# Symb0x76/ChineseChessZero

Measured on AMD Instinct MI355X. Metric: self-play MCTS simulations/sec, higher is better.
Workload: dtype u8 rules / f32 Q (reference CPU path) / f64 PUCT (net: fp16)

## Files before the change

### chinesechesszero_amd/csrc/cczero_conv_g16.h

```cpp
#pragma once
#include "cczero_conv.h"

namespace ccz {

constexpr int kG5Rows = 288;
constexpr int kG5SlabRows = 576;
constexpr int kG5SlabBytes = kG5SlabRows * 64;
constexpr int kG5WBytes = 256 * 64;
constexpr int kG5Ring = 5, kG5Ahead = 3;
constexpr int kG5AOff = kG5Ring * kG5WBytes;
constexpr int kG5Dump = kG5AOff + 2 * kG5SlabBytes;
constexpr int kG5Lds = kG5Dump + 8 * 1024;
constexpr int kG5ERow = 528;
static_assert(kG5Rows * kG5ERow <= kG5Dump, "epilogue image must fit the operand buffers");

struct G5Ctx {
    unsigned char *lds;
    const _Float16 *X, *W;
    unsigned xoff[5];
    unsigned woff;
    int zo[2], zd[2];
    int wave_dst;
    int lane16;
    int wave_dst4;
    int a_off;
    int vb[2];
    int cin, cmask;
};

__host__ __device__ constexpr bool g5_slab_tap(int t) { return t >= 1 && t <= 5; }
constexpr int kG5Split = 7;
__host__ __device__ constexpr int g5_vmcnt(int t) { return 4 + (g5_slab_tap(t) ? 1 : 0) + (g5_slab_tap(t - 1) ? 1 : 0); }

template <int T, int N> __host__ __device__ constexpr bool g5_on_board()
{
    return !((T % 3 == 0 && N == 0) || (T % 3 == 2 && N == 8));
}

__device__ __forceinline__ void g5_zero_ranks(const G5Ctx &c, int buf)
{
    int l16 = c.lane16, zero = 0;
    asm volatile("" : "+v"(l16), "+v"(zero));
    typedef int g5_int4 __attribute__((ext_vector_type(4)));
    const g5_int4 z = {zero, zero, zero, zero};
#pragma unroll
    for (int j = 0; j < 2; ++j) *(g5_int4 *)(c.lds + (l16 + (c.zo[j] + buf * c.zd[j]))) = z;
    asm volatile("s_waitcnt lgkmcnt(0)" ::: "memory");
}

template <int J>
__device__ __forceinline__ void g5_step(const G5Ctx &c, cv_f32x4 (&acc)[4][9], int chunk, int &ring_rd, int &ring_wr,
                                         cv_half8 (&a0)[4], cv_half8 (&a1)[4], cv_half8 (&b)[9])
{
    constexpr int T = J % 9, BUF = J / 9;
    constexpr int Tn = (T + 1) % 9, BUFn = (T == 8) ? 1 - BUF : BUF;
    cv_half8 (&acur)[4] = (J & 1) ? a1 : a0;
    cv_half8 (&anxt)[4] = (J & 1) ? a0 : a1;
    unsigned char *const lds = c.lds;

#define G5_CELL(N)                                                                                                        \
    {                                                                                                                     \
        if constexpr (T % 3 == 2)                                                                                         \
            b[N] = *(const cv_half8 *)(lds + c.vb[BUFn] + (9 + N + 9 * (Tn / 3 - 1)) * 1024);                             \
        if constexpr (g5_on_board<T, N>()) {                                                                              \
            constexpr int NB = N + T % 3 - 1;                                                                             \
            _Pragma("unroll") for (int i = 0; i < 4; ++i)                                                                 \
                acc[i][N] = __builtin_amdgcn_mfma_f32_16x16x32_f16(acur[i], b[NB], acc[i][N], 0, 0, 0);                   \
        }                                                                                                                 \
        __builtin_amdgcn_sched_barrier(0);                                                                                \
    }
#define G5_CELLS(LO, HI)                                                                                                  \
    if constexpr (LO <= 0 && 0 < HI) G5_CELL(0) if constexpr (LO <= 1 && 1 < HI) G5_CELL(1) if constexpr (LO <= 2 && 2 < HI) G5_CELL(2) \
    if constexpr (LO <= 3 && 3 < HI) G5_CELL(3) if constexpr (LO <= 4 && 4 < HI) G5_CELL(4) if constexpr (LO <= 5 && 5 < HI) G5_CELL(5) \
    if constexpr (LO <= 6 && 6 < HI) G5_CELL(6) if constexpr (LO <= 7 && 7 < HI) G5_CELL(7) if constexpr (LO <= 8 && 8 < HI) G5_CELL(8)
    constexpr int T2 = (T + kG5Ahead) % 9;
    const int chunk2 = (chunk + (T + kG5Ahead >= 9 ? 1 : 0)) & c.cmask;
    G5_CELLS(0, 1)
    if constexpr (g5_slab_tap(T)) {
        constexpr int pass = T - 1;
        const int nxt = (chunk + 1) & c.cmask;
        cv_glds16(c.X + (c.xoff[pass] + (unsigned)(nxt * 32)), lds + kG5AOff + (1 - BUF) * kG5SlabBytes + (pass < 4 ? pass * 8192 + c.wave_dst : c.wave_dst4));
        __builtin_amdgcn_sched_barrier(0);
    }
    G5_CELLS(1, 2)
    {
        unsigned wo = c.woff;
        asm volatile("" : "+v"(wo));
        const unsigned o = wo + (unsigned)((T2 + 9 * chunk2) * 8192);
        const unsigned o2 = o + 4096u;
        unsigned char *const d = lds + ring_wr * kG5WBytes + c.wave_dst;
        cv_glds16(c.W + o, d);
        __builtin_amdgcn_sched_barrier(0);
        G5_CELLS(2, 3)
        cv_glds16(c.W + o2, d + 8192);
        __builtin_amdgcn_sched_barrier(0);
    }
    G5_CELLS(3, kG5Split)

    ring_rd = ring_rd + 1 == kG5Ring ? 0 : ring_rd + 1;
    cv_wait_vm<g5_vmcnt(T)>();
    if constexpr (T == 7) g5_zero_ranks(c, 1 - BUF);
    __builtin_amdgcn_sched_barrier(0);
    __builtin_amdgcn_s_barrier();
    __builtin_amdgcn_sched_barrier(0);

    {
        const unsigned char *wa = lds + (ring_rd * kG5WBytes + c.a_off);
#pragma unroll
        for (int i = 0; i < 4; ++i) anxt[i] = *(const cv_half8 *)(wa + i * 1024);
        __builtin_amdgcn_sched_barrier(0);
    }
    G5_CELLS(kG5Split, 9)
    ring_wr = ring_wr + 1 == kG5Ring ? 0 : ring_wr + 1;
#undef G5_CELLS
#undef G5_CELL
}

struct G5Heads {
    const _Float16 *w32;
    const float *b32;
    _Float16 *pol, *val;
    int nb;
};

__device__ __forceinline__ void g5_heads_phase(const unsigned char *lds, int w, int lane, const G5Heads &ha, const long (&board0)[2],
                                               const int (&pos0)[2], bool skip1)
{
    const int r = lane & 15, q4 = lane >> 4;
    cv_half8 a[2][8];
#pragma unroll
    for (int m = 0; m < 2; ++m)
#pragma unroll
        for (int s = 0; s < 8; ++s) a[m][s] = *(const cv_half8 *)(ha.w32 + (m * 16 + r) * 256 + s * 32 + q4 * 8);
    const float4 b0 = *(const float4 *)(ha.b32 + 4 * q4), b1 = *(const float4 *)(ha.b32 + 16 + 4 * q4);
    for (int cell = w; cell < 18; cell += 8) {
        const unsigned char *row = lds + (cell * 16 + r) * kG5ERow + q4 * 16;
        cv_f32x4 acc0, acc1;
        acc0[0] = b0.x; acc0[1] = b0.y; acc0[2] = b0.z; acc0[3] = b0.w;
        acc1[0] = b1.x; acc1[1] = b1.y; acc1[2] = b1.z; acc1[3] = b1.w;
#pragma unroll
        for (int s = 0; s < 8; ++s) {
            const cv_half8 b = *(const cv_half8 *)(row + s * 64);
            acc0 = __builtin_amdgcn_mfma_f32_16x16x32_f16(a[0][s], b, acc0, 0, 0, 0);
            acc1 = __builtin_amdgcn_mfma_f32_16x16x32_f16(a[1][s], b, acc1, 0, 0, 0);
        }
        const int wnr = cell >= 9 ? 1 : 0, n = cell - 9 * wnr;
        const long board = board0[wnr] + r;
        if (board < ha.nb && !(skip1 && wnr)) {
            const int pos = pos0[wnr] + n;
            _Float16 *po = ha.pol + board * 1536 + pos * 17;
            _Float16 *vo = ha.val + board * 640 + pos * 7;
#pragma unroll
            for (int e = 0; e < 4; ++e) po[4 * q4 + e] = (_Float16)fmaxf(acc0[e], 0.0f);
            if (q4 == 0) {
                po[16] = (_Float16)fmaxf(acc1[0], 0.0f);
                vo[0] = (_Float16)fmaxf(acc1[1], 0.0f);
                vo[1] = (_Float16)fmaxf(acc1[2], 0.0f);
                vo[2] = (_Float16)fmaxf(acc1[3], 0.0f);
            } else if (q4 == 1) {
#pragma unroll
                for (int e = 0; e < 4; ++e) vo[3 + e] = (_Float16)fmaxf(acc1[e], 0.0f);
            }
        }
    }
}

__device__ __forceinline__ int g5_live_groups(const int *live_rows, int row0, int cap, int &first)
{
    const int part = row0 & 0xffff, n_parts = row0 >> 16;
    const int G = (*live_rows + 15) >> 4;
    const int per = (G + n_parts - 1) / n_parts;
    first = part * per;
    int live = G - first;
    live = live < 0 ? 0 : (live > per ? per : live);
    return live > cap ? cap : live;
}

template <bool RES, bool HEADS, bool ONE = false>
__device__ __forceinline__ void g5_tile(unsigned char *lds, int blk, int grid, const _Float16 *__restrict__ X, const _Float16 *__restrict__ W,
                                        const float *__restrict__ bias, const _Float16 *R,
                                        _Float16 *Y, int M, int relu, int cin, const int *live_rows, int row0, const G5Heads &ha)
{
    [[maybe_unused]] long first_board = 0;
    const int tid = threadIdx.x, lane = tid & 63;
    const int w = __builtin_amdgcn_readfirstlane(tid >> 6);
    const int r = lane & 15, q4 = lane >> 4;
    const int wm = w & 3, wn = w >> 2;
    int tiles = grid;
    if (live_rows) {
        int first;
        const int live = g5_live_groups(live_rows, row0, M / 1440, first);
        M = live * 1440;
        tiles = live * ((relu & 4) ? 4 : 5);
        if (blk >= tiles) return;
        const long off = (long)first * 1440 * kCvC;
        X += (long)first * 1440 * cin;
        if (!HEADS) Y += off;
        if (RES) R += off;
        first_board = (long)first * 16;
    }
    int tile;
    {
        const int b = blk, x = b & 7, per = tiles >> 3, rem = tiles & 7;
        tile = x * per + (x < rem ? x : rem) + (b >> 3);
    }
    tile = __builtin_amdgcn_readfirstlane((relu & 2) ? tiles - 1 - tile : tile);
    const int mid = relu & 4;
    const int k = mid ? 2 : tile % 5;
    const long p0 = mid ? (long)(tile >> 2) * 1440 + 144 + (long)(tile & 3) * kG5Rows
                        : (long)tile * kG5Rows;
    relu &= 1;

    G5Ctx c;
    c.lds = lds;
    c.X = X;
    c.W = W;
    {
        const int piece[2] = {k == 0 ? 0 : k == 4 ? (w >= 3 ? 3 : 4) : -1, (k == 0 && w == 0) ? 1 : (k == 4 && w == 3) ? 4 : -1};
#pragma unroll
        for (int j = 0; j < 2; ++j) {
            c.zo[j] = __builtin_amdgcn_readfirstlane(piece[j] >= 0 ? kG5AOff + piece[j] * 8192 + w * 1024 : kG5Dump + w * 1024);
            c.zd[j] = __builtin_amdgcn_readfirstlane(piece[j] >= 0 ? kG5SlabBytes : 0);
        }
    }
    c.wave_dst = w * 1024;
    c.lane16 = lane * 16;
    c.wave_dst4 = (w < 4 ? 4 : 3) * 8192 + w * 1024;
    c.cin = cin;
    c.cmask = ONE ? 0 : (cin >> 5) - 1;
    {
#pragma unroll
        for (int it = 0; it < 5; ++it) {
            const int piece = (it < 4 || w < 4) ? it * 512 + tid : 3 * 512 + tid;
            const int sr = piece >> 2, pos = piece & 3;
            const int schunk = pos ^ ((0 - (sr >> 2)) & 3);
            long p = p0 - 144 + sr;
            p = p < 0 ? 0 : (p > (long)M - 1 ? (long)M - 1 : p);
            c.xoff[it] = (unsigned)(p * cin + schunk * 8);
        }
        c.woff = (unsigned)(tid * 8);
    }
#pragma unroll
    for (int it = 0; it < 5; ++it) cv_glds16(X + c.xoff[it], lds + kG5AOff + (it < 4 ? it * 8192 + c.wave_dst : c.wave_dst4));
#pragma unroll
    for (int u = 0; u < kG5Ahead; ++u) {
        const unsigned o = c.woff + (unsigned)(u * 8192);
        unsigned char *d = lds + u * kG5WBytes + c.wave_dst;
        cv_glds16(W + o, d);
        cv_glds16(W + (o + 4096u), d + 8192);
    }
    const int lane1 = r * 64 + ((q4 ^ ((0 - (r >> 2)) & 3)) << 4);
    c.a_off = wm * 4096 + lane1;
    c.vb[0] = kG5AOff + wn * 9 * 1024 + lane1;
    c.vb[1] = c.vb[0] + kG5SlabBytes;

    cv_f32x4 acc[4][9];
#pragma unroll
    for (int i = 0; i < 4; ++i) {
        const float4 bv = *(const float4 *)(bias + wm * 64 + i * 16 + 4 * q4);
#pragma unroll
        for (int n = 0; n < 9; ++n) {
            acc[i][n][0] = bv.x; acc[i][n][1] = bv.y; acc[i][n][2] = bv.z; acc[i][n][3] = bv.w;
        }
    }

    cv_wait_vm<4>();
    g5_zero_ranks(c, 0);
    asm volatile("s_waitcnt lgkmcnt(0)" ::: "memory");
    __builtin_amdgcn_sched_barrier(0);
    __builtin_amdgcn_s_barrier();
    __builtin_amdgcn_sched_barrier(0);

    int ring_rd = 0, ring_wr = kG5Ahead;
    cv_half8 a0[4], a1[4], b[9];
#pragma unroll
    for (int i = 0; i < 4; ++i) a0[i] = *(const cv_half8 *)(lds + c.a_off + i * 1024);
#pragma unroll
    for (int n = 0; n < 9; ++n) b[n] = *(const cv_half8 *)(lds + c.vb[0] + (9 + n - 9) * 1024);
#define G5_S(j) g5_step<j>(c, acc, chunk + (j) / 9, ring_rd, ring_wr, a0, a1, b)
    if constexpr (ONE) {
        const int chunk = 0;
        G5_S(0); G5_S(1); G5_S(2); G5_S(3); G5_S(4); G5_S(5); G5_S(6); G5_S(7); G5_S(8);
    } else {
        for (int chunk = 0; chunk <= c.cmask; chunk += 2) {
            G5_S(0); G5_S(1); G5_S(2); G5_S(3); G5_S(4); G5_S(5); G5_S(6); G5_S(7); G5_S(8);
            G5_S(9); G5_S(10); G5_S(11); G5_S(12); G5_S(13); G5_S(14); G5_S(15); G5_S(16); G5_S(17);
        }
    }
#undef G5_S
    cv_wait_vm<0>();

    __builtin_amdgcn_sched_barrier(0);
    __builtin_amdgcn_s_barrier();
    __builtin_amdgcn_sched_barrier(0);
#pragma unroll
    for (int i = 0; i < 4; ++i) {
        const int col = wm * 64 + i * 16 + 4 * q4;
#pragma unroll
        for (int n = 0; n < 9; ++n) {
            cv_half4 o;
            o[0] = (_Float16)acc[i][n][0];
            o[1] = (_Float16)acc[i][n][1];
            o[2] = (_Float16)acc[i][n][2];
            o[3] = (_Float16)acc[i][n][3];
            *(cv_half4 *)(lds + ((wn * 9 + n) * 16 + r) * kG5ERow + col * 2) = o;
        }
    }
    const int prow = lane >> 5, piece = lane & 31;
    const long pbase = p0 + w * 36 + prow;
    cv_half8 rv[18];
    if (RES) {
#pragma unroll
        for (int it = 0; it < 18; ++it) rv[it] = *(const cv_half8 *)(R + (pbase + it * 2) * kCvC + piece * 8);
    }
    asm volatile("s_waitcnt lgkmcnt(0)" ::: "memory");
    __builtin_amdgcn_sched_barrier(0);
    __builtin_amdgcn_s_barrier();
    __builtin_amdgcn_sched_barrier(0);
    {
        const cv_half8 zero = (cv_half8)(_Float16)0;
        unsigned char *eb = lds + (w * 36 + prow) * kG5ERow + piece * 16;
#pragma unroll
        for (int it = 0; it < 18; ++it) {
            cv_half8 v = *(const cv_half8 *)(eb + it * 2 * kG5ERow);
            if (RES) v = v + rv[it];
            if (relu) v = __builtin_elementwise_max(v, zero);
            if constexpr (HEADS) *(cv_half8 *)(eb + it * 2 * kG5ERow) = v;
            else *(cv_half8 *)(Y + (pbase + it * 2) * kCvC + piece * 8) = v;
        }
    }
    if constexpr (HEADS) {
        asm volatile("s_waitcnt lgkmcnt(0)" ::: "memory");
        __builtin_amdgcn_sched_barrier(0);
        __builtin_amdgcn_s_barrier();
        __builtin_amdgcn_sched_barrier(0);
        const long grp = p0 / 1440;
        const int rank0 = (int)((p0 - grp * 1440) / 144);
        const long board0[2] = {first_board + grp * 16, first_board + grp * 16};
        const int pos0[2] = {rank0 * 9, rank0 * 9 + 9};
        g5_heads_phase(lds, w, lane, ha, board0, pos0, false);
    }
}

template <bool RES>
__global__ __launch_bounds__(512) void k_conv3x3_g16(const _Float16 *__restrict__ X, const _Float16 *__restrict__ W,
                                                         const float *__restrict__ bias, const _Float16 *R,
                                                         _Float16 *Y, int M, int relu, int cin, const int *live_rows, int row0)
{
    __shared__ __attribute__((aligned(16))) unsigned char lds[kG5Lds];
    g5_tile<RES, false>(lds, blockIdx.x, gridDim.x, X, W, bias, R, Y, M, relu, cin, live_rows, row0, G5Heads{});
}

__global__ __launch_bounds__(512) void k_conv3x3_g16_stem(const _Float16 *__restrict__ X, const _Float16 *__restrict__ W,
                                                            const float *__restrict__ bias, _Float16 *Y, int M, int relu, int cin,
                                                            const int *live_rows, int row0)
{
    __shared__ __attribute__((aligned(16))) unsigned char lds[kG5Lds];
    g5_tile<false, false, true>(lds, blockIdx.x, gridDim.x, X, W, bias, nullptr, Y, M, relu, cin, live_rows, row0, G5Heads{});
}

__global__ __launch_bounds__(512) void k_conv3x3_g16_heads(const _Float16 *__restrict__ X, const _Float16 *__restrict__ W,
                                                             const float *__restrict__ bias, const _Float16 *R, _Float16 *Y, int M,
                                                             int relu, int cin, const int *live_rows, int row0, G5Heads ha)
{
    __shared__ __attribute__((aligned(16))) unsigned char lds[kG5Lds];
    if (live_rows) ha.nb = *live_rows;
    g5_tile<true, true>(lds, blockIdx.x, gridDim.x, X, W, bias, R, Y, M, relu, cin, live_rows, row0, ha);
}

__global__ __launch_bounds__(256) void k_pack_conv_weights_g16(const cv_half8 *__restrict__ w, cv_half8 *__restrict__ wp, int cin)
{
    const int n = 256 * 9 * (cin >> 3);
    const int i = blockIdx.x * 256 + threadIdx.x;
    if (i >= n) return;
    const int pos = i & 3, co = (i >> 2) & 255, h = i >> 10, tap = h % 9, c32 = h / 9;
    const int chunk = pos ^ ((0 - (co >> 2)) & 3);
    wp[i] = w[(co * 9 + tap) * (cin >> 3) + c32 * 4 + chunk];
}

}
```

### chinesechesszero_amd/csrc/cczero_conv_g16e.h

```cpp
#pragma once
#include "cczero_conv_g16.h"

namespace ccz {

__host__ __device__ constexpr int g5e_nslab(int h) { return h == 0 ? 2 : h == 1 ? 2 : h == 2 ? 1 : 0; }
__host__ __device__ constexpr int g5e_vmcnt(int h) { return 4 + g5e_nslab(h) + g5e_nslab((h + 5) % 6); }

template <int J>
__device__ __forceinline__ void g5e_step(const G5Ctx &c, cv_f32x4 (&acc)[4][9], int chunk, int &ring_rd, int &ring_wr,
                                          cv_half8 (&a0)[4], cv_half8 (&a1)[4], cv_half8 (&b)[9], int toff)
{
    constexpr int H = J % 6, BUF = J / 6;
    constexpr int Hn = (H + 1) % 6, BUFn = (H == 5) ? 1 - BUF : BUF;
    cv_half8 (&acur)[4] = (J & 1) ? a1 : a0;
    cv_half8 (&anxt)[4] = (J & 1) ? a0 : a1;
    unsigned char *const lds = c.lds;
#define G5E_CELL(N)                                                                                                       \
    {                                                                                                                     \
        if constexpr (H % 3 == 2)                                                                                         \
            b[N] = *(const cv_half8 *)(lds + c.vb[BUFn] + ((Hn / 3) * 9 + N) * 1024);                                     \
        if constexpr (g5_on_board<H, N>()) {                                                                              \
            constexpr int NB = N + H % 3 - 1;                                                                             \
            _Pragma("unroll") for (int i = 0; i < 4; ++i)                                                                 \
                acc[i][N] = __builtin_amdgcn_mfma_f32_16x16x32_f16(acur[i], b[NB], acc[i][N], 0, 0, 0);                   \
        }                                                                                                                 \
        __builtin_amdgcn_sched_barrier(0);                                                                                \
    }
#define G5E_CELLS(LO, HI)                                                                                                 \
    if constexpr (LO <= 0 && 0 < HI) G5E_CELL(0) if constexpr (LO <= 1 && 1 < HI) G5E_CELL(1) if constexpr (LO <= 2 && 2 < HI) G5E_CELL(2) \
    if constexpr (LO <= 3 && 3 < HI) G5E_CELL(3) if constexpr (LO <= 4 && 4 < HI) G5E_CELL(4) if constexpr (LO <= 5 && 5 < HI) G5E_CELL(5) \
    if constexpr (LO <= 6 && 6 < HI) G5E_CELL(6) if constexpr (LO <= 7 && 7 < HI) G5E_CELL(7) if constexpr (LO <= 8 && 8 < HI) G5E_CELL(8)
    constexpr int H2 = (H + kG5Ahead) % 6;
    const int chunk2 = (chunk + (H + kG5Ahead >= 6 ? 1 : 0)) & c.cmask;
    G5E_CELLS(0, 1)
    if constexpr (g5e_nslab(H) > 0) {
        const int nxt = (chunk + 1) & c.cmask;
        constexpr int p0 = H * 2;
        cv_glds16(c.X + (c.xoff[p0] + (unsigned)(nxt * 32)), lds + kG5AOff + (1 - BUF) * kG5SlabBytes + (p0 < 4 ? p0 * 8192 + c.wave_dst : c.wave_dst4));
        if constexpr (g5e_nslab(H) > 1)
            cv_glds16(c.X + (c.xoff[p0 + 1] + (unsigned)(nxt * 32)), lds + kG5AOff + (1 - BUF) * kG5SlabBytes + ((p0 + 1) * 8192 + c.wave_dst));
        __builtin_amdgcn_sched_barrier(0);
    }
    G5E_CELLS(1, 2)
    {
        unsigned wo = c.woff;
        asm volatile("" : "+v"(wo));
        const unsigned o = wo + (unsigned)((H2 + toff + 9 * chunk2) * 8192);
        const unsigned o2 = o + 4096u;
        unsigned char *const d = lds + ring_wr * kG5WBytes + c.wave_dst;
        cv_glds16(c.W + o, d);
        __builtin_amdgcn_sched_barrier(0);
        G5E_CELLS(2, 3)
        cv_glds16(c.W + o2, d + 8192);
        __builtin_amdgcn_sched_barrier(0);
    }
    G5E_CELLS(3, kG5Split)

    ring_rd = ring_rd + 1 == kG5Ring ? 0 : ring_rd + 1;
    cv_wait_vm<g5e_vmcnt(H)>();
    __builtin_amdgcn_sched_barrier(0);
    __builtin_amdgcn_s_barrier();
    __builtin_amdgcn_sched_barrier(0);

    {
        const unsigned char *wa = lds + (ring_rd * kG5WBytes + c.a_off);
#pragma unroll
        for (int i = 0; i < 4; ++i) anxt[i] = *(const cv_half8 *)(wa + i * 1024);
        __builtin_amdgcn_sched_barrier(0);
    }
    G5E_CELLS(kG5Split, 9)
    ring_wr = ring_wr + 1 == kG5Ring ? 0 : ring_wr + 1;
#undef G5E_CELLS
#undef G5E_CELL
}

template <bool RES, bool HEADS>
__device__ __forceinline__ void g5e_tile(unsigned char *lds, int blk, const _Float16 *__restrict__ X, const _Float16 *__restrict__ W,
                                         const float *__restrict__ bias, const _Float16 *R, _Float16 *Y, int M,
                                         int relu, int cin, const int *live_rows, int row0, const G5Heads &ha)
{
    [[maybe_unused]] long first_board = 0;
    const int tid = threadIdx.x, lane = tid & 63;
    const int w = __builtin_amdgcn_readfirstlane(tid >> 6);
    const int r = lane & 15, q4 = lane >> 4;
    const int wm = w & 3, wn = w >> 2;
    int groups = M / 1440;
    if (live_rows) {
        int first;
        groups = g5_live_groups(live_rows, row0, groups, first);
        const long off = (long)first * 1440 * kCvC;
        X += (long)first * 1440 * cin;
        if (!HEADS) Y += off;
        if (RES) R += off;
        first_board = (long)first * 16;
    }
    const int e = __builtin_amdgcn_readfirstlane(blk);
    if (e >= 2 * ((groups + 1) >> 1)) return;
    const int side = e & 1, gA = (e >> 1) * 2;
    const bool dup = gA + 1 >= groups;
    const int gB = dup ? gA : gA + 1;
    const int toff = __builtin_amdgcn_readfirstlane(side ? 0 : 3);
    const long srcA = (long)gA * 1440 + (side ? 8 : 0) * 144;
    const long srcB = (long)gB * 1440 + (side ? 8 : 0) * 144;
    const long outA = (long)gA * 1440 + (side ? 9 : 0) * 144;
    const long outB = (long)gB * 1440 + (side ? 9 : 0) * 144;
    relu &= 1;

    G5Ctx c;
    c.lds = lds;
    c.X = X;
    c.W = W;
    c.wave_dst = w * 1024;
    c.lane16 = lane * 16;
    c.wave_dst4 = (w < 4 ? 4 : 3) * 8192 + w * 1024;
    c.cin = cin;
    c.cmask = (cin >> 5) - 1;
    {
#pragma unroll
        for (int it = 0; it < 5; ++it) {
            const int piece = (it < 4 || w < 4) ? it * 512 + tid : 3 * 512 + tid;
            const int sr = piece >> 2, pos = piece & 3;
            const int schunk = pos ^ ((0 - (sr >> 2)) & 3);
            const long p = sr < 288 ? srcA + sr : srcB + (sr - 288);
            c.xoff[it] = (unsigned)(p * cin + schunk * 8);
        }
        c.woff = (unsigned)(tid * 8);
    }
#pragma unroll
    for (int it = 0; it < 5; ++it) cv_glds16(X + c.xoff[it], lds + kG5AOff + (it < 4 ? it * 8192 + c.wave_dst : c.wave_dst4));
#pragma unroll
    for (int u = 0; u < kG5Ahead; ++u) {
        const unsigned o = c.woff + (unsigned)((u + toff) * 8192);
        unsigned char *d = lds + u * kG5WBytes + c.wave_dst;
        cv_glds16(W + o, d);
        cv_glds16(W + (o + 4096u), d + 8192);
    }
    const int lane1 = r * 64 + ((q4 ^ ((0 - (r >> 2)) & 3)) << 4);
    c.a_off = wm * 4096 + lane1;
    c.vb[0] = kG5AOff + wn * 18 * 1024 + lane1;
    c.vb[1] = c.vb[0] + kG5SlabBytes;

    cv_f32x4 acc[4][9];
#pragma unroll
    for (int i = 0; i < 4; ++i) {
        const float4 bv = *(const float4 *)(bias + wm * 64 + i * 16 + 4 * q4);
#pragma unroll
        for (int n = 0; n < 9; ++n) {
            acc[i][n][0] = bv.x; acc[i][n][1] = bv.y; acc[i][n][2] = bv.z; acc[i][n][3] = bv.w;
        }
    }

    cv_wait_vm<4>();
    __builtin_amdgcn_sched_barrier(0);
    __builtin_amdgcn_s_barrier();
    __builtin_amdgcn_sched_barrier(0);

    int ring_rd = 0, ring_wr = kG5Ahead;
    cv_half8 a0[4], a1[4], b[9];
#pragma unroll
    for (int i = 0; i < 4; ++i) a0[i] = *(const cv_half8 *)(lds + c.a_off + i * 1024);
#pragma unroll
    for (int n = 0; n < 9; ++n) b[n] = *(const cv_half8 *)(lds + c.vb[0] + n * 1024);
    for (int chunk = 0; chunk <= c.cmask; chunk += 2) {
#define G5E_S(j) g5e_step<j>(c, acc, chunk + (j) / 6, ring_rd, ring_wr, a0, a1, b, toff)
        G5E_S(0); G5E_S(1); G5E_S(2); G5E_S(3); G5E_S(4); G5E_S(5);
        G5E_S(6); G5E_S(7); G5E_S(8); G5E_S(9); G5E_S(10); G5E_S(11);
#undef G5E_S
    }
    cv_wait_vm<0>();

    __builtin_amdgcn_sched_barrier(0);
    __builtin_amdgcn_s_barrier();
    __builtin_amdgcn_sched_barrier(0);
#pragma unroll
    for (int i = 0; i < 4; ++i) {
        const int col = wm * 64 + i * 16 + 4 * q4;
#pragma unroll
        for (int n = 0; n < 9; ++n) {
            cv_half4 o;
            o[0] = (_Float16)acc[i][n][0];
            o[1] = (_Float16)acc[i][n][1];
            o[2] = (_Float16)acc[i][n][2];
            o[3] = (_Float16)acc[i][n][3];
            *(cv_half4 *)(lds + ((wn * 9 + n) * 16 + r) * kG5ERow + col * 2) = o;
        }
    }
    const int prow = lane >> 5, piece = lane & 31;
    const long pbase = (w < 4 ? outA : outB) + (w & 3) * 36 + prow;
    const bool store = !(dup && w >= 4);
    cv_half8 rv[18];
    if (RES) {
#pragma unroll
        for (int it = 0; it < 18; ++it) rv[it] = *(const cv_half8 *)(R + (pbase + it * 2) * kCvC + piece * 8);
    }
    asm volatile("s_waitcnt lgkmcnt(0)" ::: "memory");
    __builtin_amdgcn_sched_barrier(0);
    __builtin_amdgcn_s_barrier();
    __builtin_amdgcn_sched_barrier(0);
    if (store) {
        const cv_half8 zero = (cv_half8)(_Float16)0;
        unsigned char *eb = lds + (w * 36 + prow) * kG5ERow + piece * 16;
#pragma unroll
        for (int it = 0; it < 18; ++it) {
            cv_half8 v = *(const cv_half8 *)(eb + it * 2 * kG5ERow);
            if (RES) v = v + rv[it];
            if (relu) v = __builtin_elementwise_max(v, zero);
            if constexpr (HEADS) *(cv_half8 *)(eb + it * 2 * kG5ERow) = v;
            else *(cv_half8 *)(Y + (pbase + it * 2) * kCvC + piece * 8) = v;
        }
    }
    if constexpr (HEADS) {
        asm volatile("s_waitcnt lgkmcnt(0)" ::: "memory");
        __builtin_amdgcn_sched_barrier(0);
        __builtin_amdgcn_s_barrier();
        __builtin_amdgcn_sched_barrier(0);
        const long board0[2] = {first_board + (long)gA * 16, first_board + (long)gB * 16};
        const int pos0[2] = {side ? 81 : 0, side ? 81 : 0};
        g5_heads_phase(lds, w, lane, ha, board0, pos0, dup);
    }
}

template <bool RES>
__global__ __launch_bounds__(512) void k_conv3x3_g16_edge(const _Float16 *__restrict__ X, const _Float16 *__restrict__ W,
                                                            const float *__restrict__ bias, const _Float16 *R, _Float16 *Y, int M,
                                                            int relu, int cin, const int *live_rows, int row0)
{
    __shared__ __attribute__((aligned(16))) unsigned char lds[kG5Lds];
    g5e_tile<RES, false>(lds, blockIdx.x, X, W, bias, R, Y, M, relu, cin, live_rows, row0, G5Heads{});
}

__global__ __launch_bounds__(512) void k_conv3x3_g16_edge_heads(const _Float16 *__restrict__ X, const _Float16 *__restrict__ W,
                                                                  const float *__restrict__ bias, const _Float16 *R, _Float16 *Y,
                                                                  int M, int relu, int cin, const int *live_rows, int row0, G5Heads ha)
{
    __shared__ __attribute__((aligned(16))) unsigned char lds[kG5Lds];
    if (live_rows) ha.nb = *live_rows;
    g5e_tile<true, true>(lds, blockIdx.x, X, W, bias, R, Y, M, relu, cin, live_rows, row0, ha);
}

template <bool RES>
__global__ __launch_bounds__(512) void k_conv3x3_g16_one(const _Float16 *__restrict__ X, const _Float16 *__restrict__ W,
                                                           const float *__restrict__ bias, const _Float16 *R, _Float16 *Y, int M,
                                                           int relu, int cin, const int *live_rows, int row0)
{
    __shared__ __attribute__((aligned(16))) unsigned char lds[kG5Lds];
    int groups = M / 1440;
    if (live_rows) {
        int first;
        groups = g5_live_groups(live_rows, row0, groups, first);
    }
    const int mid = groups * 4, blk = blockIdx.x;
    if (blk < mid) g5_tile<RES, false>(lds, blk, mid, X, W, bias, R, Y, M, relu | 4, cin, live_rows, row0, G5Heads{});
    else g5e_tile<RES, false>(lds, blk - mid, X, W, bias, R, Y, M, relu, cin, live_rows, row0, G5Heads{});
}

}
```

### profiles/conv_stamps.py

```python
import ctypes as C
import json
import os
import sys

import numpy as np
import torch

ROOT = os.path.dirname(os.path.dirname(os.path.abspath(__file__)))
sys.path.insert(0, ROOT)
from chinesechesszero_amd import _lib

_lib.LIB_PATH = os.path.join(ROOT, "build", "diag", "libcczero_stamps.so")


def main():
    B = int(sys.argv[1]) if len(sys.argv) > 1 else 4096
    dev = torch.device("cuda:0")
    g = torch.Generator(device="cpu").manual_seed(1)
    cl = torch.channels_last
    x = (torch.randn(B, 256, 10, 9, generator=g) * 0.5).to(dev).half().contiguous(memory_format=cl)
    w = (torch.randn(256, 256, 3, 3, generator=g) * 0.03).to(dev).half().contiguous(memory_format=cl)
    bias = (torch.randn(256, generator=g) * 0.1).to(dev)
    y = torch.empty_like(x)
    L = _lib.lib()
    L.ccz_debug_conv_stamps.restype = C.c_int
    L.ccz_debug_conv_stamps.argtypes = [C.c_void_p]
    out = {}
    for name, dbg in [("plain", 0)] + [("dbg%d" % int(v), int(v)) for v in os.environ.get("CONV_DBG", "").split(",") if v]:
        relu = 1 | (dbg << 8)
        for _ in range(200):
            _lib.check(L.ccz_conv3x3_c256_f16(C.c_void_p(torch.cuda.current_stream().cuda_stream), C.c_void_p(x.data_ptr()), C.c_void_p(w.data_ptr()),
                                              C.c_void_p(bias.data_ptr()), None, C.c_void_p(y.data_ptr()), B * 90, relu))
        torch.cuda.synchronize()
        st = np.zeros(2048 * 2 * 16, np.uint64)
        _lib.check(L.ccz_debug_conv_stamps(st.ctypes.data_as(C.c_void_p)))
        tiles = min(2048, (B * 90 + 255) // 256)
        st = st.reshape(2048, 2, 16)[:tiles].astype(np.int64)
        loop = st[:, :, 1] - st[:, :, 0]
        real = st[:, :, 4] - st[:, :, 3]
        rec = {"tiles_sampled": int(tiles), "loop_cycles_median": float(np.median(loop)), "loop_cycles_per_halfstep": float(np.median(loop)) / 72,
               "prologue_cycles_median": float(np.median(st[:, :, 0] - st[:, :, 10])), "epilogue_cycles_median": float(np.median(st[:, :, 2] - st[:, :, 1])),
               "clock_ghz_median": float(np.median(loop / np.maximum(real, 1)) * 0.1)}
        out[name] = rec
    print(json.dumps(out, indent=1))


if __name__ == "__main__":
    main()
```

Measured before the change: 193,000.

## Peel last conv chunk to skip wasted prefetch and overlap residual loads

The last chunk pair of the g16 and g16-edge conv K-loops is peeled into tail steps. These steps no longer issue wrap-around slab and weight prefetches, use smaller vmcnt waits, and drop the final barrier. The full vm drain before the epilogue is gone, and residual loads are issued before the accumulator-to-LDS image writes so they overlap. Stamp instrumentation and an MFMA-only probe build are added behind compile flags, and the lane index is recomputed for the epilogue. The risk is in the hand-tuned wait counts: if one is wrong, the epilogue could read LDS data that has not arrived yet.

```diff
diff --git a/chinesechesszero_amd/csrc/cczero_conv_g16.h b/chinesechesszero_amd/csrc/cczero_conv_g16.h
--- a/chinesechesszero_amd/csrc/cczero_conv_g16.h
+++ b/chinesechesszero_amd/csrc/cczero_conv_g16.h
@@ -28,9 +28,35 @@
     int cin, cmask;
 };
 
+#ifdef CCZ_STAMPS
+#define G5_STAMP_DECL unsigned long long g5_st[9] = {}
+#define G5_STAMP(i) g5_st[i] = cv_stamp()
+#define G5_STAMP_REAL(i) (g5_st[i] = __builtin_amdgcn_s_memrealtime(), __builtin_amdgcn_s_waitcnt(0xC07F))
+#define G5_STAMP_DRAIN() asm volatile("s_waitcnt vmcnt(0)" ::: "memory")
+#define G5_STAMP_WRITE()                                                                                                  \
+    if (blockIdx.x < 2048 && (w & 3) == 0 && elane == 0) {   \
+        unsigned long long *o_ = g_cv_stamps + (blockIdx.x * 2 + (w >> 2)) * 16;                                          \
+        _Pragma("unroll") for (int i_ = 0; i_ < 9; ++i_) o_[i_] = g5_st[i_];                                              \
+    }
+#else
+#define G5_STAMP_DECL
+#define G5_STAMP(i)
+#define G5_STAMP_REAL(i)
+#define G5_STAMP_DRAIN()
+#define G5_STAMP_WRITE()
+#endif
+
+#ifdef CCZ_G16_MFMA_ONLY
+constexpr bool kG5MfmaOnly = true;
+#else
+constexpr bool kG5MfmaOnly = false;
+#endif
+
 __host__ __device__ constexpr bool g5_slab_tap(int t) { return t >= 1 && t <= 5; }
 constexpr int kG5Split = 7;
 __host__ __device__ constexpr int g5_vmcnt(int t) { return 4 + (g5_slab_tap(t) ? 1 : 0) + (g5_slab_tap(t - 1) ? 1 : 0); }
+constexpr int kG5LastW = 8 - kG5Ahead;
+__host__ __device__ constexpr int g5_vmcnt_tail(int t) { return (t <= kG5LastW ? 2 : 0) + (t - 1 <= kG5LastW ? 2 : 0); }
 
 template <int T, int N> __host__ __device__ constexpr bool g5_on_board()
 {
@@ -48,19 +74,28 @@
     asm volatile("s_waitcnt lgkmcnt(0)" ::: "memory");
 }
 
-template <int J>
+__device__ __forceinline__ int g5_lane_again()
+{
+    int l;
+    asm volatile("v_mbcnt_lo_u32_b32 %0, -1, 0\n\tv_mbcnt_hi_u32_b32 %0, -1, %0" : "=v"(l));
+    return l;
+}
+
+template <int J, bool TAIL = false>
 __device__ __forceinline__ void g5_step(const G5Ctx &c, cv_f32x4 (&acc)[4][9], int chunk, int &ring_rd, int &ring_wr,
                                          cv_half8 (&a0)[4], cv_half8 (&a1)[4], cv_half8 (&b)[9])
 {
     constexpr int T = J % 9, BUF = J / 9;
     constexpr int Tn = (T + 1) % 9, BUFn = (T == 8) ? 1 - BUF : BUF;
+    constexpr bool LAST = (TAIL && T == 8) || kG5MfmaOnly;
+    constexpr bool WDMA = !(TAIL && T > kG5LastW) && !kG5MfmaOnly;
     cv_half8 (&acur)[4] = (J & 1) ? a1 : a0;
     cv_half8 (&anxt)[4] = (J & 1) ? a0 : a1;
     unsigned char *const lds = c.lds;
 
 #define G5_CELL(N)                                                                                                        \
     {                                                                                                                     \
-        if constexpr (T % 3 == 2)                                                                                         \
+        if constexpr (T % 3 == 2 && !LAST)                                                                                \
             b[N] = *(const cv_half8 *)(lds + c.vb[BUFn] + (9 + N + 9 * (Tn / 3 - 1)) * 1024);                             \
         if constexpr (g5_on_board<T, N>()) {                                                                              \
             constexpr int NB = N + T % 3 - 1;                                                                             \
@@ -76,14 +111,14 @@
     constexpr int T2 = (T + kG5Ahead) % 9;
     const int chunk2 = (chunk + (T + kG5Ahead >= 9 ? 1 : 0)) & c.cmask;
     G5_CELLS(0, 1)
-    if constexpr (g5_slab_tap(T)) {
+    if constexpr (g5_slab_tap(T) && !TAIL && !kG5MfmaOnly) {
         constexpr int pass = T - 1;
         const int nxt = (chunk + 1) & c.cmask;
         cv_glds16(c.X + (c.xoff[pass] + (unsigned)(nxt * 32)), lds + kG5AOff + (1 - BUF) * kG5SlabBytes + (pass < 4 ? pass * 8192 + c.wave_dst : c.wave_dst4));
         __builtin_amdgcn_sched_barrier(0);
     }
     G5_CELLS(1, 2)
-    {
+    if constexpr (WDMA) {
         unsigned wo = c.woff;
         asm volatile("" : "+v"(wo));
         const unsigned o = wo + (unsigned)((T2 + 9 * chunk2) * 8192);
@@ -94,17 +129,20 @@
         G5_CELLS(2, 3)
         cv_glds16(c.W + o2, d + 8192);
         __builtin_amdgcn_sched_barrier(0);
+    } else {
+        G5_CELLS(2, 3)
     }
     G5_CELLS(3, kG5Split)
 
-    ring_rd = ring_rd + 1 == kG5Ring ? 0 : ring_rd + 1;
-    cv_wait_vm<g5_vmcnt(T)>();
-    if constexpr (T == 7) g5_zero_ranks(c, 1 - BUF);
-    __builtin_amdgcn_sched_barrier(0);
-    __builtin_amdgcn_s_barrier();
-    __builtin_amdgcn_sched_barrier(0);
-
-    {
+    if constexpr (!LAST) {
+        ring_rd = ring_rd + 1 == kG5Ring ? 0 : ring_rd + 1;
+        if constexpr (TAIL) cv_wait_vm<g5_vmcnt_tail(T)>();
+        else cv_wait_vm<g5_vmcnt(T)>();
+        if constexpr (T == 7 && !TAIL) g5_zero_ranks(c, 1 - BUF);
+        __builtin_amdgcn_sched_barrier(0);
+        __builtin_amdgcn_s_barrier();
+        __builtin_amdgcn_sched_barrier(0);
+
         const unsigned char *wa = lds + (ring_rd * kG5WBytes + c.a_off);
 #pragma unroll
         for (int i = 0; i < 4; ++i) anxt[i] = *(const cv_half8 *)(wa + i * 1024);
@@ -184,6 +222,8 @@
     [[maybe_unused]] long first_board = 0;
     const int tid = threadIdx.x, lane = tid & 63;
     const int w = __builtin_amdgcn_readfirstlane(tid >> 6);
+    G5_STAMP_DECL;
+    G5_STAMP(0);
     const int r = lane & 15, q4 = lane >> 4;
     const int wm = w & 3, wn = w >> 2;
     int tiles = grid;
@@ -277,25 +317,47 @@
     for (int i = 0; i < 4; ++i) a0[i] = *(const cv_half8 *)(lds + c.a_off + i * 1024);
 #pragma unroll
     for (int n = 0; n < 9; ++n) b[n] = *(const cv_half8 *)(lds + c.vb[0] + (9 + n - 9) * 1024);
+    if constexpr (kG5MfmaOnly) {
+#pragma unroll
+        for (int i = 0; i < 4; ++i) a1[i] = a0[i];
+    }
+    G5_STAMP(1);
+    G5_STAMP_REAL(7);
 #define G5_S(j) g5_step<j>(c, acc, chunk + (j) / 9, ring_rd, ring_wr, a0, a1, b)
+#define G5_T(j) g5_step<j, true>(c, acc, chunk + (j) / 9, ring_rd, ring_wr, a0, a1, b)
     if constexpr (ONE) {
         const int chunk = 0;
-        G5_S(0); G5_S(1); G5_S(2); G5_S(3); G5_S(4); G5_S(5); G5_S(6); G5_S(7); G5_S(8);
+        G5_T(0); G5_T(1); G5_T(2); G5_T(3); G5_T(4); G5_T(5); G5_T(6); G5_T(7); G5_T(8);
     } else {
-        for (int chunk = 0; chunk <= c.cmask; chunk += 2) {
+        int chunk = 0;
+        for (; chunk < c.cmask - 1; chunk += 2) {
             G5_S(0); G5_S(1); G5_S(2); G5_S(3); G5_S(4); G5_S(5); G5_S(6); G5_S(7); G5_S(8);
             G5_S(9); G5_S(10); G5_S(11); G5_S(12); G5_S(13); G5_S(14); G5_S(15); G5_S(16); G5_S(17);
         }
+        G5_S(0); G5_S(1); G5_S(2); G5_S(3); G5_S(4); G5_S(5); G5_S(6); G5_S(7); G5_S(8);
+        G5_T(9); G5_T(10); G5_T(11); G5_T(12); G5_T(13); G5_T(14); G5_T(15); G5_T(16); G5_T(17);
     }
 #undef G5_S
-    cv_wait_vm<0>();
+#undef G5_T
+    G5_STAMP(2);
+    G5_STAMP_REAL(8);
+    G5_STAMP(3);
 
     __builtin_amdgcn_sched_barrier(0);
     __builtin_amdgcn_s_barrier();
     __builtin_amdgcn_sched_barrier(0);
+    const int elane = g5_lane_again(), er = elane & 15, eq4 = elane >> 4;
+    const int prow = elane >> 5, piece = elane & 31;
+    const long pbase = p0 + w * 36 + prow;
+    cv_half8 rv[18];
+    if (RES) {
+#pragma unroll
+        for (int it = 0; it < 18; ++it) rv[it] = *(const cv_half8 *)(R + (pbase + it * 2) * kCvC + piece * 8);
+    }
+    __builtin_amdgcn_sched_barrier(0);
 #pragma unroll
     for (int i = 0; i < 4; ++i) {
-        const int col = wm * 64 + i * 16 + 4 * q4;
+        const int col = wm * 64 + i * 16 + 4 * eq4;
 #pragma unroll
         for (int n = 0; n < 9; ++n) {
             cv_half4 o;
@@ -303,20 +365,16 @@
             o[1] = (_Float16)acc[i][n][1];
             o[2] = (_Float16)acc[i][n][2];
             o[3] = (_Float16)acc[i][n][3];
-            *(cv_half4 *)(lds + ((wn * 9 + n) * 16 + r) * kG5ERow + col * 2) = o;
-        }
-    }
-    const int prow = lane >> 5, piece = lane & 31;
-    const long pbase = p0 + w * 36 + prow;
-    cv_half8 rv[18];
-    if (RES) {
-#pragma unroll
-        for (int it = 0; it < 18; ++it) rv[it] = *(const cv_half8 *)(R + (pbase + it * 2) * kCvC + piece * 8);
+            *(cv_half4 *)(lds + ((wn * 9 + n) * 16 + er) * kG5ERow + col * 2) = o;
+        }
     }
     asm volatile("s_waitcnt lgkmcnt(0)" ::: "memory");
     __builtin_amdgcn_sched_barrier(0);
     __builtin_amdgcn_s_barrier();
     __builtin_amdgcn_sched_barrier(0);
+    G5_STAMP(4);
+    G5_STAMP_DRAIN();
+    G5_STAMP(5);
     {
         const cv_half8 zero = (cv_half8)(_Float16)0;
         unsigned char *eb = lds + (w * 36 + prow) * kG5ERow + piece * 16;
@@ -329,6 +387,8 @@
             else *(cv_half8 *)(Y + (pbase + it * 2) * kCvC + piece * 8) = v;
         }
     }
+    G5_STAMP(6);
+    G5_STAMP_WRITE();
     if constexpr (HEADS) {
         asm volatile("s_waitcnt lgkmcnt(0)" ::: "memory");
         __builtin_amdgcn_sched_barrier(0);
@@ -338,7 +398,7 @@
         const int rank0 = (int)((p0 - grp * 1440) / 144);
         const long board0[2] = {first_board + grp * 16, first_board + grp * 16};
         const int pos0[2] = {rank0 * 9, rank0 * 9 + 9};
-        g5_heads_phase(lds, w, lane, ha, board0, pos0, false);
+        g5_heads_phase(lds, w, elane, ha, board0, pos0, false);
     }
 }
 
diff --git a/chinesechesszero_amd/csrc/cczero_conv_g16e.h b/chinesechesszero_amd/csrc/cczero_conv_g16e.h
--- a/chinesechesszero_amd/csrc/cczero_conv_g16e.h
+++ b/chinesechesszero_amd/csrc/cczero_conv_g16e.h
@@ -5,19 +5,23 @@
 
 __host__ __device__ constexpr int g5e_nslab(int h) { return h == 0 ? 2 : h == 1 ? 2 : h == 2 ? 1 : 0; }
 __host__ __device__ constexpr int g5e_vmcnt(int h) { return 4 + g5e_nslab(h) + g5e_nslab((h + 5) % 6); }
-
-template <int J>
+constexpr int kG5ELastW = 5 - kG5Ahead;
+__host__ __device__ constexpr int g5e_vmcnt_tail(int h) { return (h <= kG5ELastW ? 2 : 0) + (h - 1 <= kG5ELastW ? 2 : 0); }
+
+template <int J, bool TAIL = false>
 __device__ __forceinline__ void g5e_step(const G5Ctx &c, cv_f32x4 (&acc)[4][9], int chunk, int &ring_rd, int &ring_wr,
                                           cv_half8 (&a0)[4], cv_half8 (&a1)[4], cv_half8 (&b)[9], int toff)
 {
     constexpr int H = J % 6, BUF = J / 6;
     constexpr int Hn = (H + 1) % 6, BUFn = (H == 5) ? 1 - BUF : BUF;
+    constexpr bool LAST = (TAIL && H == 5) || kG5MfmaOnly;
+    constexpr bool WDMA = !(TAIL && H > kG5ELastW) && !kG5MfmaOnly;
     cv_half8 (&acur)[4] = (J & 1) ? a1 : a0;
     cv_half8 (&anxt)[4] = (J & 1) ? a0 : a1;
     unsigned char *const lds = c.lds;
 #define G5E_CELL(N)                                                                                                       \
     {                                                                                                                     \
-        if constexpr (H % 3 == 2)                                                                                         \
+        if constexpr (H % 3 == 2 && !LAST)                                                                                \
             b[N] = *(const cv_half8 *)(lds + c.vb[BUFn] + ((Hn / 3) * 9 + N) * 1024);                                     \
         if constexpr (g5_on_board<H, N>()) {                                                                              \
             constexpr int NB = N + H % 3 - 1;                                                                             \
@@ -33,7 +37,7 @@
     constexpr int H2 = (H + kG5Ahead) % 6;
     const int chunk2 = (chunk + (H + kG5Ahead >= 6 ? 1 : 0)) & c.cmask;
     G5E_CELLS(0, 1)
-    if constexpr (g5e_nslab(H) > 0) {
+    if constexpr (g5e_nslab(H) > 0 && !TAIL && !kG5MfmaOnly) {
         const int nxt = (chunk + 1) & c.cmask;
         constexpr int p0 = H * 2;
         cv_glds16(c.X + (c.xoff[p0] + (unsigned)(nxt * 32)), lds + kG5AOff + (1 - BUF) * kG5SlabBytes + (p0 < 4 ? p0 * 8192 + c.wave_dst : c.wave_dst4));
@@ -42,7 +46,7 @@
         __builtin_amdgcn_sched_barrier(0);
     }
     G5E_CELLS(1, 2)
-    {
+    if constexpr (WDMA) {
         unsigned wo = c.woff;
         asm volatile("" : "+v"(wo));
         const unsigned o = wo + (unsigned)((H2 + toff + 9 * chunk2) * 8192);
@@ -53,16 +57,19 @@
         G5E_CELLS(2, 3)
         cv_glds16(c.W + o2, d + 8192);
         __builtin_amdgcn_sched_barrier(0);
+    } else {
+        G5E_CELLS(2, 3)
     }
     G5E_CELLS(3, kG5Split)
 
-    ring_rd = ring_rd + 1 == kG5Ring ? 0 : ring_rd + 1;
-    cv_wait_vm<g5e_vmcnt(H)>();
-    __builtin_amdgcn_sched_barrier(0);
-    __builtin_amdgcn_s_barrier();
-    __builtin_amdgcn_sched_barrier(0);
-
-    {
+    if constexpr (!LAST) {
+        ring_rd = ring_rd + 1 == kG5Ring ? 0 : ring_rd + 1;
+        if constexpr (TAIL) cv_wait_vm<g5e_vmcnt_tail(H)>();
+        else cv_wait_vm<g5e_vmcnt(H)>();
+        __builtin_amdgcn_sched_barrier(0);
+        __builtin_amdgcn_s_barrier();
+        __builtin_amdgcn_sched_barrier(0);
+
         const unsigned char *wa = lds + (ring_rd * kG5WBytes + c.a_off);
 #pragma unroll
         for (int i = 0; i < 4; ++i) anxt[i] = *(const cv_half8 *)(wa + i * 1024);
@@ -82,6 +89,8 @@
     [[maybe_unused]] long first_board = 0;
     const int tid = threadIdx.x, lane = tid & 63;
     const int w = __builtin_amdgcn_readfirstlane(tid >> 6);
+    G5_STAMP_DECL;
+    G5_STAMP(0);
     const int r = lane & 15, q4 = lane >> 4;
     const int wm = w & 3, wn = w >> 2;
     int groups = M / 1440;
@@ -161,20 +170,43 @@
     for (int i = 0; i < 4; ++i) a0[i] = *(const cv_half8 *)(lds + c.a_off + i * 1024);
 #pragma unroll
     for (int n = 0; n < 9; ++n) b[n] = *(const cv_half8 *)(lds + c.vb[0] + n * 1024);
-    for (int chunk = 0; chunk <= c.cmask; chunk += 2) {
+    if constexpr (kG5MfmaOnly) {
+#pragma unroll
+        for (int i = 0; i < 4; ++i) a1[i] = a0[i];
+    }
+    G5_STAMP(1);
+    G5_STAMP_REAL(7);
 #define G5E_S(j) g5e_step<j>(c, acc, chunk + (j) / 6, ring_rd, ring_wr, a0, a1, b, toff)
+#define G5E_T(j) g5e_step<j, true>(c, acc, chunk + (j) / 6, ring_rd, ring_wr, a0, a1, b, toff)
+    int chunk = 0;
+    for (; chunk < c.cmask - 1; chunk += 2) {
         G5E_S(0); G5E_S(1); G5E_S(2); G5E_S(3); G5E_S(4); G5E_S(5);
         G5E_S(6); G5E_S(7); G5E_S(8); G5E_S(9); G5E_S(10); G5E_S(11);
+    }
+    G5E_S(0); G5E_S(1); G5E_S(2); G5E_S(3); G5E_S(4); G5E_S(5);
+    G5E_T(6); G5E_T(7); G5E_T(8); G5E_T(9); G5E_T(10); G5E_T(11);
 #undef G5E_S
-    }
-    cv_wait_vm<0>();
+#undef G5E_T
+    G5_STAMP(2);
+    G5_STAMP_REAL(8);
+    G5_STAMP(3);
 
     __builtin_amdgcn_sched_barrier(0);
     __builtin_amdgcn_s_barrier();
     __builtin_amdgcn_sched_barrier(0);
+    const int elane = g5_lane_again(), er = elane & 15, eq4 = elane >> 4;
+    const int prow = elane >> 5, piece = elane & 31;
+    const long pbase = (w < 4 ? outA : outB) + (w & 3) * 36 + prow;
+    const bool store = !(dup && w >= 4);
+    cv_half8 rv[18];
+    if (RES) {
+#pragma unroll
+        for (int it = 0; it < 18; ++it) rv[it] = *(const cv_half8 *)(R + (pbase + it * 2) * kCvC + piece * 8);
+    }
+    __builtin_amdgcn_sched_barrier(0);
 #pragma unroll
     for (int i = 0; i < 4; ++i) {
-        const int col = wm * 64 + i * 16 + 4 * q4;
+        const int col = wm * 64 + i * 16 + 4 * eq4;
 #pragma unroll
         for (int n = 0; n < 9; ++n) {
             cv_half4 o;
@@ -182,21 +214,16 @@
             o[1] = (_Float16)acc[i][n][1];
             o[2] = (_Float16)acc[i][n][2];
             o[3] = (_Float16)acc[i][n][3];
-            *(cv_half4 *)(lds + ((wn * 9 + n) * 16 + r) * kG5ERow + col * 2) = o;
-        }
-    }
-    const int prow = lane >> 5, piece = lane & 31;
-    const long pbase = (w < 4 ? outA : outB) + (w & 3) * 36 + prow;
-    const bool store = !(dup && w >= 4);
-    cv_half8 rv[18];
-    if (RES) {
-#pragma unroll
-        for (int it = 0; it < 18; ++it) rv[it] = *(const cv_half8 *)(R + (pbase + it * 2) * kCvC + piece * 8);
+            *(cv_half4 *)(lds + ((wn * 9 + n) * 16 + er) * kG5ERow + col * 2) = o;
+        }
     }
     asm volatile("s_waitcnt lgkmcnt(0)" ::: "memory");
     __builtin_amdgcn_sched_barrier(0);
     __builtin_amdgcn_s_barrier();
     __builtin_amdgcn_sched_barrier(0);
+    G5_STAMP(4);
+    G5_STAMP_DRAIN();
+    G5_STAMP(5);
     if (store) {
         const cv_half8 zero = (cv_half8)(_Float16)0;
         unsigned char *eb = lds + (w * 36 + prow) * kG5ERow + piece * 16;
@@ -209,6 +236,8 @@
             else *(cv_half8 *)(Y + (pbase + it * 2) * kCvC + piece * 8) = v;
         }
     }
+    G5_STAMP(6);
+    G5_STAMP_WRITE();
     if constexpr (HEADS) {
         asm volatile("s_waitcnt lgkmcnt(0)" ::: "memory");
         __builtin_amdgcn_sched_barrier(0);
@@ -216,7 +245,7 @@
         __builtin_amdgcn_sched_barrier(0);
         const long board0[2] = {first_board + (long)gA * 16, first_board + (long)gB * 16};
         const int pos0[2] = {side ? 81 : 0, side ? 81 : 0};
-        g5_heads_phase(lds, w, lane, ha, board0, pos0, dup);
+        g5_heads_phase(lds, w, elane, ha, board0, pos0, dup);
     }
 }
 
diff --git a/profiles/conv_stamps.py b/profiles/conv_stamps.py
--- a/profiles/conv_stamps.py
+++ b/profiles/conv_stamps.py
@@ -10,10 +10,68 @@
 sys.path.insert(0, ROOT)
 from chinesechesszero_amd import _lib
 
-_lib.LIB_PATH = os.path.join(ROOT, "build", "diag", "libcczero_stamps.so")
+_lib.LIB_PATH = os.environ.get("CONV_STAMPS_LIB") or os.path.join(ROOT, "build", "diag", "libcczero_stamps.so")
+
+G16_STAMPS = ["entry", "first_mfma", "loop_end", "dma_drained", "image_barrier", "residual_arrived", "last_store_issued"]
+
+
+def g16(B):
+    dev = torch.device("cuda:0")
+    g = torch.Generator(device="cpu").manual_seed(1)
+    x = torch.relu(torch.randn(B * 90, 256, generator=g) * 0.5).to(dev).half()
+    r = (torch.randn(B * 90, 256, generator=g) * 0.5).to(dev).half()
+    w = (torch.randn(256, 3, 3, 256, generator=g) * 0.03).to(dev).half()
+    bias = (torch.randn(256, generator=g) * 0.1).to(dev)
+    y = torch.empty_like(x)
+    L = _lib.lib()
+    L.ccz_debug_conv_stamps.restype = C.c_int
+    L.ccz_debug_conv_stamps.argtypes = [C.c_void_p]
+    wp = torch.empty(8, 9, 256, 32, dtype=torch.float16, device=dev)
+    stream = C.c_void_p(torch.cuda.current_stream().cuda_stream)
+    _lib.check(L.ccz_pack_conv_weights_g16_f16(stream, C.c_void_p(w.data_ptr()), C.c_void_p(wp.data_ptr()), 256))
+    flags = _lib.CONV_RELU | _lib.CONV_G16 | _lib.CONV_G16_EDGE_TILES | _lib.CONV_G16_ONE_LAUNCH
+    groups = B // 16
+    n_mid, n_edge = 4 * groups, 2 * ((groups + 1) // 2)
+    out = {"library": os.path.basename(_lib.LIB_PATH), "boards": B, "stamps": G16_STAMPS}
+
+    def launch(res):
+        _lib.check(L.ccz_conv3x3_c256_f16(stream, C.c_void_p(x.data_ptr()), C.c_void_p(wp.data_ptr()), C.c_void_p(bias.data_ptr()),
+                                          C.c_void_p(r.data_ptr()) if res else None, C.c_void_p(y.data_ptr()), B * 90, flags))
+
+    for res in (False, True):
+        import time
+        t0 = time.time()
+        while time.time() - t0 < 2.0:
+            for _ in range(200):
+                launch(res)
+            torch.cuda.synchronize()
+        reps = []
+        for _ in range(5):
+            e0, e1 = torch.cuda.Event(enable_timing=True), torch.cuda.Event(enable_timing=True)
+            e0.record()
+            for _ in range(200):
+                launch(res)
+            e1.record()
+            torch.cuda.synchronize()
+            reps.append(e0.elapsed_time(e1) * 1000 / 200)
+        st = np.zeros(2048 * 2 * 16, np.uint64)
+        _lib.check(L.ccz_debug_conv_stamps(st.ctypes.data_as(C.c_void_p)))
+        st = st.reshape(2048, 2, 16).astype(np.int64)
+        rec = {"layer_us": [round(v, 2) for v in reps]}
+        for name, lo, hi in (("middle", 0, min(n_mid, 2048)), ("edge", min(n_mid, 2048), min(n_mid + n_edge, 2048))):
+            t = st[lo:hi].reshape(-1, 16)
+            ghz = np.median((t[:, 2] - t[:, 1]) / np.maximum(t[:, 8] - t[:, 7], 1)) * 0.1
+            seg = {G16_STAMPS[i] + "->" + G16_STAMPS[i + 1]: float(np.median(t[:, i + 1] - t[:, i])) for i in range(6)}
+            rec[name] = {"tiles": int(hi - lo), "cycles_median": seg, "tile_cycles_median": float(np.median(t[:, 6] - t[:, 0])),
+                         "clock_ghz_in_loop": round(float(ghz), 3), "tile_us": round(float(np.median(t[:, 6] - t[:, 0]) / ghz / 1000), 2),
+                         "p90_cycles": {G16_STAMPS[i] + "->" + G16_STAMPS[i + 1]: float(np.percentile(t[:, i + 1] - t[:, i], 90)) for i in range(6)}}
+        out["residual" if res else "no_residual"] = rec
+    print(json.dumps(out, indent=1))
 
 
 def main():
+    if len(sys.argv) > 1 and sys.argv[1] == "g16":
+        return g16(int(sys.argv[2]) if len(sys.argv) > 2 else 4096)
     B = int(sys.argv[1]) if len(sys.argv) > 1 else 4096
     dev = torch.device("cuda:0")
     g = torch.Generator(device="cpu").manual_seed(1)
```

After: 194,800, median of 6. No clear change (+0.9%).
